# yangdongchao/RSTnet

Hardware: AMD Instinct MI355X
Metric: codec+LM audio frames/sec (24 kHz, 12.5 Hz tokens) at batch=1 and batch=64; RVQ code-index exact-match (higher is better)
Workload: dtype f32 (large GEMMs: operands as three bf16 planes, six bf16 matrix-instruction products per fp32 product, f32 accumulate); 1 GPU; MimiCodec encode->RVQ(8x2048x256)->decode, BASELINE.json configs[1]; batch_per_gpu=64, weights=random-init (rstnet_amd.synth seed 0), parallelism=replica x1, utterances sharded, RCCL weight broadcast only

## Files before the change

### rstnet_amd/csrc/b3_common.h

```cpp
#pragma once
#include "rst_common.h"

typedef short bf16x8 __attribute__((ext_vector_type(8)));
typedef unsigned u32x2 __attribute__((ext_vector_type(2)));
typedef unsigned u32x4 __attribute__((ext_vector_type(4)));
typedef float f32x2 __attribute__((ext_vector_type(2)));
typedef __bf16 bf16x2_t __attribute__((ext_vector_type(2)));

__device__ __forceinline__ unsigned b3_peel(f32x2& v) {
    const unsigned h = __builtin_bit_cast(unsigned, __builtin_convertvector(v, bf16x2_t));
    v[0] -= __uint_as_float(h << 16);
    v[1] -= __uint_as_float(h & 0xffff0000u);
    return h;
}

constexpr int B3_SH_ROWS = 128;

struct B3SharedTile {
    int b, t0;
    long m0, mlim;
};
struct B3SharedRow {
    unsigned ao;
    int klo, kn;
};

__host__ __device__ __forceinline__ constexpr int b3_shared_step(int R) { return B3_SH_ROWS - (R - 1); }
__host__ __device__ __forceinline__ constexpr int b3_shared_tiles_per_utt(int T_out, int R) { return (T_out + b3_shared_step(R) - 1) / b3_shared_step(R); }

__host__ __device__ __forceinline__ B3SharedTile b3_shared_tile(int mt, int R, int T_out) {
    const int tpu = b3_shared_tiles_per_utt(T_out, R), step = b3_shared_step(R);
    B3SharedTile t;
    t.b = mt / tpu;
    t.t0 = (mt - t.b * tpu) * step;
    t.m0 = (long)t.b * T_out + t.t0;
    t.mlim = (long)t.b * T_out + (t.t0 + step < T_out ? t.t0 + step : T_out);
    return t;
}

__host__ __device__ __forceinline__ B3SharedRow b3_shared_row(const B3SharedTile& t, int r, int R, int G, int TC, long x_bstride, int lk) {
    const long g = (long)t.t0 + r - (R - 1);
    const long f0 = g * G;
    B3SharedRow o;
    o.klo = 0;
    if (g < 0 || f0 >= TC) {
        o.kn = 0;
        o.ao = (unsigned)(lk * 4);
    } else {
        const long left = TC - f0;
        o.kn = (int)((left < G ? left : (long)G) / 16);
        o.ao = (unsigned)(((long)t.b * x_bstride + f0 + lk) * 4);
    }
    return o;
}

__host__ __device__ __forceinline__ unsigned b3_shared_load_offset(const B3SharedRow& row, int kt, bool& ok) {
    ok = (unsigned)kt < (unsigned)row.kn;
    return row.ao + (ok ? (unsigned)kt : 0u) * 64u;
}

#define B3_QA {2, 0, 1, 1, 0, 0}
#define B3_QB {0, 2, 1, 0, 1, 0}
```

### rstnet_amd/csrc/gemm_win.hip

```cpp
#include <algorithm>
#include "rst_common.h"
#include "rst_kernels.h"
#include "b3_common.h"

namespace {

constexpr int BK = 32;

template <int TM, int TN, bool FULL = false>
__device__ __forceinline__ void gw_epilogue(const GemmWinParams& p, const f32x16 (&acc)[TM][TN], int m0w, int n0w, int M, int lane) {
    const bool has_res = p.res != nullptr;
#pragma unroll
    for (int j = 0; j < TN; ++j) {
        const int n = n0w + j * 32 + (lane & 31);
        const bool n_ok = FULL || n < p.N;
        const float bias = (p.bias && n_ok) ? p.bias[n] : 0.0f;
        const float scale = (p.scale && n_ok) ? p.scale[n] : 1.0f;
#pragma unroll
        for (int i = 0; i < TM; ++i) {
            const int mb = m0w + i * 32 + 4 * (lane >> 5);
            const long o = (long)mb * p.ldy + n;
            float r[16];
#pragma unroll
            for (int e = 0; e < 16; ++e) {
                const int dm = (e & 3) + 8 * (e >> 2);
                r[e] = (has_res && n_ok && (FULL || mb + dm < M)) ? p.res[o + (long)dm * p.ldy] : 0.0f;
            }
#pragma unroll
            for (int e = 0; e < 16; ++e) {
                const int dm = (e & 3) + 8 * (e >> 2);
                float v = acc[i][j][e] + bias;
                if (p.act_out == 1) v = rst_gelu(v);
                if (has_res) v = r[e] + scale * v;
                if (p.act_out == 2) v = rst_elu(v);
                if (n_ok && (FULL || mb + dm < M)) p.y[o + (long)dm * p.ldy] = v;
            }
        }
    }
}

template <int TM, int TN, int WM, int WN, bool VEC, bool ELU, int KB, bool FAST>
__device__ __forceinline__ void gw_tile(const GemmWinParams& p, const int tile, const int m0, const int n0, float* smem) {
    constexpr int BM = 32 * TM * WM;
    constexpr int BN = 32 * TN * WN;
    constexpr int LDS_LD = KB + 4;
    constexpr int RP = 1024 / KB;
    constexpr int RA = BM / RP;
    constexpr int RB = BN / RP;
    static_assert(BM % RP == 0 && BN % RP == 0, "tile smaller than one staging pass");
    float* As = smem;
    float* Bs = smem + 2 * BM * LDS_LD;

    const int tid = threadIdx.x;
    const int lane = tid & 63;
    const int wave = tid >> 6;
    const int wm = wave / WN, wn = wave % WN;

    const int M = p.B * p.T_out;
    const int TC = p.T_in * p.C;
    const int PC = p.P * p.C;

    const int lrow = tid / (KB / 4);
    const int lk = (tid % (KB / 4)) * 4;
    long a_off[RA];
    long h_off[RA];
    int a_f0[RA];
    int a_klo[RA], a_khi[RA];
    bool a_ok[RA];
#pragma unroll
    for (int j = 0; j < RA; ++j) {
        const int m = m0 + lrow + RP * j;
        a_ok[j] = m < M;
        const int mm = a_ok[j] ? m : 0;
        const int b = mm / p.T_out;
        const int t = mm - b * p.T_out;
        a_off[j] = (long)b * p.x_bstride;
        h_off[j] = (long)b * PC;
        a_f0[j] = (t * p.S - p.P) * p.C;
        a_klo[j] = a_ok[j] ? max(0, -a_f0[j]) : 0x7fffffff;
        a_khi[j] = a_ok[j] ? min(p.K, TC - a_f0[j]) : 0;
    }

    f32x4 ra[RA], rb[RB];

    auto load_elem_a = [&](int j, int f) -> float {
        float v = 0.0f;
        if (f >= 0) {
            if (f < TC) v = p.x[a_off[j] + f];
            else if (p.pad_mode == 1) v = p.x[a_off[j] + TC - p.C + f % p.C];
        } else if (p.hist) {
            v = p.hist[h_off[j] + PC + f];
        } else if (p.pad_mode == 1) {
            int c = f % p.C;
            if (c < 0) c += p.C;
            v = p.x[a_off[j] + c];
        }
        return v;
    };

    typedef int i32x4 __attribute__((ext_vector_type(4)));
    int ma[RA], mb[RB];
    auto masked_load = [&](const float* src, bool ok, int& m) -> f32x4 {
        m = ok ? -1 : 0;
        asm volatile("" : "+v"(m));
        return *reinterpret_cast<const f32x4*>(ok ? src : p.w);
    };
    auto apply_mask = [&](const f32x4 v, const int m) -> f32x4 {
        const i32x4 b = __builtin_bit_cast(i32x4, v) & m;
        return __builtin_bit_cast(f32x4, b);
    };
    auto load_tiles = [&](int kt) {
        const int k = kt * KB + lk;
#pragma unroll
        for (int j = 0; j < RA; ++j) {
            if (VEC) {
                const int f = a_f0[j] + k;
                bool ok = a_ok[j] && k < p.K;
                const float* src = p.x + a_off[j] + f;
                if (f < 0) {
                    if (p.hist) {
                        src = p.hist + h_off[j] + PC + f;
                    } else if (p.pad_mode == 1) {
                        int c = f % p.C;
                        if (c < 0) c += p.C;
                        src = p.x + a_off[j] + c;
                    } else {
                        ok = false;
                    }
                } else if (f >= TC) {
                    if (p.pad_mode == 1) src = p.x + a_off[j] + TC - p.C + f % p.C;
                    else ok = false;
                }
                ra[j] = masked_load(src, ok, ma[j]);
            } else {
                ma[j] = -1;
                f32x4 v = {0.f, 0.f, 0.f, 0.f};
                if (a_ok[j]) {
#pragma unroll
                    for (int e = 0; e < 4; ++e)
                        if (k + e < p.K) v[e] = load_elem_a(j, a_f0[j] + k + e);
                }
                ra[j] = v;
            }
        }
#pragma unroll
        for (int j = 0; j < RB; ++j) {
            const int n = n0 + lrow + RP * j;
            const float* wp = p.w + (long)n * p.K + k;
            if (VEC) {
                rb[j] = masked_load(wp, n < p.N && k < p.K, mb[j]);
            } else {
                mb[j] = -1;
                f32x4 v = {0.f, 0.f, 0.f, 0.f};
                if (n < p.N) {
#pragma unroll
                    for (int e = 0; e < 4; ++e)
                        if (k + e < p.K) v[e] = wp[e];
                }
                rb[j] = v;
            }
        }
    };

    auto store_tiles = [&](int buf, const bool masked = true) {
        float* a = As + buf * BM * LDS_LD;
        float* b = Bs + buf * BN * LDS_LD;
#pragma unroll
        for (int j = 0; j < RA; ++j) {
            f32x4 v = (VEC && masked) ? apply_mask(ra[j], ma[j]) : ra[j];
            if (ELU) {
                v[0] = rst_elu(v[0]); v[1] = rst_elu(v[1]); v[2] = rst_elu(v[2]); v[3] = rst_elu(v[3]);
            }
            *reinterpret_cast<f32x4*>(a + (lrow + RP * j) * LDS_LD + lk) = v;
        }
#pragma unroll
        for (int j = 0; j < RB; ++j)
            *reinterpret_cast<f32x4*>(b + (lrow + RP * j) * LDS_LD + lk) = (VEC && masked) ? apply_mask(rb[j], mb[j]) : rb[j];
    };

    f32x16 acc[TM][TN];
#pragma unroll
    for (int i = 0; i < TM; ++i)
#pragma unroll
        for (int j = 0; j < TN; ++j)
#pragma unroll
            for (int e = 0; e < 16; ++e) acc[i][j][e] = 0.0f;

    const int nk_all = (p.K + KB - 1) / KB;
    const int nsplit = FAST ? (int)gridDim.y : 1;
    const int per_split = (nk_all + nsplit - 1) / nsplit;
// ... 159 lines not shown
    const int tiles_n = (p.N + BN - 1) / BN;
    const int nk = p.K / KB;
    const bool k_ok = p.K % KB == 0;

    const int xcd = blockIdx.x & 7;
    const int first = gw_xcd_first(tiles, xcd);
    const int count = gw_xcd_first(tiles, xcd + 1) - first;
    const int stride = ((int)gridDim.x + 7 - xcd) >> 3;
    int l = blockIdx.x >> 3;
    if (l >= count) return;

    struct Ctx {
        const float* ap[RA];
        unsigned bo[RB];
    };
    auto setup = [&](int m0, int n0, Ctx& c) -> bool {
        bool interior = k_ok && m0 + BM <= M && n0 + BN <= p.N;
#pragma unroll
        for (int j = 0; j < RA; ++j) {
            const int m = min(m0 + lrow + RP * j, M - 1);
            const int b = m / p.T_out;
            const int t = m - b * p.T_out;
            const int f0 = (t * p.S - p.P) * p.C;
            interior = interior && f0 >= 0 && f0 + p.K <= TC;
            c.ap[j] = p.x + (long)b * p.x_bstride + f0 + lk;
        }
#pragma unroll
        for (int j = 0; j < RB; ++j) c.bo[j] = (unsigned)min(n0 + lrow + RP * j, p.N - 1) * (unsigned)p.K + lk;
        return __syncthreads_and(interior);
    };

    f32x4 ra[RA], rb[RB];
    auto issue = [&](const Ctx& c, int kt) {
#pragma unroll
        for (int j = 0; j < RA; ++j) ra[j] = *reinterpret_cast<const f32x4*>(c.ap[j] + kt * KB);
#pragma unroll
        for (int j = 0; j < RB; ++j) rb[j] = *reinterpret_cast<const f32x4*>(p.w + c.bo[j] + kt * KB);
    };
    auto store_tiles = [&](int buf) {
        float* a = As + buf * BM * LDS_LD;
        float* b = Bs + buf * BN * LDS_LD;
#pragma unroll
        for (int j = 0; j < RA; ++j) {
            f32x4 v = ra[j];
            if (ELU) {
                v[0] = rst_elu(v[0]); v[1] = rst_elu(v[1]); v[2] = rst_elu(v[2]); v[3] = rst_elu(v[3]);
            }
            *reinterpret_cast<f32x4*>(a + (lrow + RP * j) * LDS_LD + lk) = v;
        }
#pragma unroll
        for (int j = 0; j < RB; ++j)
            *reinterpret_cast<f32x4*>(b + (lrow + RP * j) * LDS_LD + lk) = rb[j];
    };

    f32x16 acc[TM][TN];
    auto clear = [&]() {
#pragma unroll
        for (int i = 0; i < TM; ++i)
#pragma unroll
            for (int j = 0; j < TN; ++j)
#pragma unroll
                for (int e = 0; e < 16; ++e) acc[i][j][e] = 0.0f;
    };
    auto mma_tile = [&](int buf, int ks0, int ks1) {
        const float* a = As + buf * BM * LDS_LD + (wm * TM * 32 + frag_row) * LDS_LD + frag_k;
        const float* b = Bs + buf * BN * LDS_LD + (wn * TN * 32 + frag_row) * LDS_LD + frag_k;
#pragma unroll
        for (int ks = ks0; ks < ks1; ++ks) {
            f32x4 fa[TM], fb[TN];
#pragma unroll
            for (int i = 0; i < TM; ++i) fa[i] = *reinterpret_cast<const f32x4*>(a + i * 32 * LDS_LD + ks * 8);
#pragma unroll
            for (int j = 0; j < TN; ++j) fb[j] = *reinterpret_cast<const f32x4*>(b + j * 32 * LDS_LD + ks * 8);
#pragma unroll
            for (int e = 0; e < 4; ++e)
#pragma unroll
                for (int i = 0; i < TM; ++i)
#pragma unroll
                    for (int j = 0; j < TN; ++j)
                        acc[i][j] = __builtin_amdgcn_mfma_f32_32x32x2f32(fa[i][e], fb[j][e], acc[i][j], 0, 0, 0);
        }
    };
    auto step = [&](const Ctx& c, int kt, int buf) {
        if (DBG == 5) {
#pragma unroll
            for (int e = 0; e < 4 * (KB / 8); ++e)
#pragma unroll
                for (int i = 0; i < TM; ++i)
#pragma unroll
                    for (int j = 0; j < TN; ++j)
                        acc[i][j] = __builtin_amdgcn_mfma_f32_32x32x2f32(ra[0][e & 3], rb[0][e & 3], acc[i][j], 0, 0, 0);
            return;
        }
        store_tiles(buf ^ 1);
        if (DBG != 1) issue(c, kt);
        __builtin_amdgcn_sched_barrier(0);
        mma_tile(buf, 0, KB / 8);
        __syncthreads();
    };
    auto prime = [&](const Ctx& c, int buf) {
        issue(c, 0);
        store_tiles(buf);
        issue(c, 1);
        __syncthreads();
    };

    Ctx c, cn;
    int tile = first + l;
    int m0 = (tile / tiles_n) * BM, n0 = (tile % tiles_n) * BN;
    bool fast = nk >= 2 && setup(m0, n0, c);
    int buf = 0;
    if (fast) prime(c, 0);
    for (;;) {
        const bool has_next = l + stride < count;
        const int tile_n = tile + stride;
        const int m0n = (tile_n / tiles_n) * BM, n0n = (tile_n % tiles_n) * BN;
        bool fast_n = false;
        if (fast) {
            clear();
            int lkt = 2;
            for (int kt = 0; kt < nk; ++kt) {
                if (lkt == nk) {
                    lkt = 0;
                    if (has_next) {
                        fast_n = setup(m0n, n0n, cn);
                        if (fast_n) c = cn;
                    }
                }
                step(c, lkt, buf);
                ++lkt;
                buf ^= 1;
            }
            gw_epilogue<TM, TN, true>(p, acc, m0 + wm * TM * 32, n0 + wn * TN * 32, M, lane);
        } else {
            gw_tile<TM, TN, WM, WN, true, ELU, KB, false>(p, tile, m0, n0, smem);
            if (has_next) fast_n = nk >= 2 && setup(m0n, n0n, c);
        }
        if (!has_next) break;
        if (fast_n && !fast) prime(c, buf);
        fast = fast_n;
        l += stride;
        tile = tile_n;
        m0 = m0n;
        n0 = n0n;
    }
}


constexpr int B3_SETS_A = 4;
constexpr int B3_SETS_B = 2;
constexpr int B3_KB = 16;
constexpr int B3_RS = 24;
constexpr int B3_WTILE = 3 * 128 * B3_KB;

template <int V>
struct b3_int { static constexpr int value = V; };

__host__ __device__ __forceinline__ constexpr int b3_row(int g) { return (g & ~7) | (2 * (g & 3) + ((g >> 2) & 1)); }
__host__ __device__ __forceinline__ constexpr int b3_slot(int r) { return (r & ~7) | (((r & 7) >> 1) + 4 * (r & 1)); }

template <bool ELU, bool MASK, int NWN, int DBG = 0, bool BUFL = true, bool DIRW = false>
__global__ __launch_bounds__(128 * NWN) __attribute__((amdgpu_waves_per_eu(2, 2))) void gemm_win_b3_stream_kernel(const GemmWinParams p, const int tiles) {
    constexpr int TM = 2, TN = 2;
    constexpr int NT = 128 * NWN;
    constexpr int BM = 128, BN = 64 * NWN;
    constexpr int RA = 512 / NT;
    constexpr int A_PLANE = BM * B3_RS, W_PLANE = DIRW ? 0 : BN * B3_RS;
    constexpr int BUF = 3 * (A_PLANE + W_PLANE);
    constexpr int NSA = B3_SETS_A, NSB = B3_SETS_B;
    static_assert(NSA == 4 && NSB == 2, "the rotation below is written out for four activation sets and two weight sets");
    static_assert(NWN == 2 || NWN == 4, "two or four waves along N");
    extern __shared__ __attribute__((aligned(16))) float smem[];
    short* const lds = reinterpret_cast<short*>(smem);

    const int tid = threadIdx.x;
    const int lane = tid & 63;
    const int wave = tid >> 6;
    const int wm = wave / NWN, wn = wave % NWN;
    const int lrow = b3_row(tid >> 2);
    const int lk = (tid & 3) * 4;
    const int frag_row = lane & 31;
    const int frag_k = (lane >> 5) * 8;

    const int M = p.B * p.T_out;
    const int TC = p.T_in * p.C;
    const int tiles_n = (p.N + BN - 1) / BN;
    const int nk = p.K / B3_KB;

    const int xcd = blockIdx.x & 7;
    const int first = gw_xcd_first(tiles, xcd);
    const int count = gw_xcd_first(tiles, xcd + 1) - first;
    const int stride = ((int)gridDim.x + 7 - xcd) >> 3;
    int l = blockIdx.x >> 3;
    if (l >= count) return;

    struct Ctx {
        unsigned ao[RA];
        int klo[RA], kn[RA];
    };
    auto setup = [&](int m0, Ctx& c) {
#pragma unroll
        for (int j = 0; j < RA; ++j) {
            const int m = m0 + lrow + (NT / 4) * j;
            const int mm = min(m, M - 1);
            const int b = mm / p.T_out;
            const int t = mm - b * p.T_out;
            const int f0 = (t * p.S - p.P) * p.C;
            long off = (long)b * p.x_bstride + f0 + lk;
            if (MASK) {
                int klo = max(0, -f0) / B3_KB, khi = min(p.K, TC - f0) / B3_KB;
                if (m >= M || klo >= khi) {
                    klo = khi = 0;
                    off = lk;
                }
                c.klo[j] = klo;
                c.kn[j] = khi - klo;
                off += (long)klo * B3_KB;
            }
            c.ao[j] = (unsigned)(off * 4);
        }
    };
    auto w_tile = [&](int n0) {
        return DIRW ? (unsigned)(n0 / 32) * (unsigned)nk * 3072u : (unsigned)(n0 / 128) * (unsigned)nk * (unsigned)(B3_WTILE * 2);
    };
    const unsigned wo = DIRW ? (unsigned)(wn * TN) * (unsigned)nk * 3072u + (unsigned)lane * 16u
                             : (unsigned)(((long)(tid >> 8) * nk * B3_WTILE + (tid & 255) * 8) * 2);
    const unsigned wo_blk = (unsigned)nk * 3072u;

    f32x4 ra[NSA][RA];
    int rm[NSA][RA];
    u32x4 rb[NSB][3];
    u32x4 rw[NSB][TN][3];
    const int a_dst = lrow * B3_RS + lk;
    const int b_dst = 3 * A_PLANE + ((tid >> 8) * 128 + b3_row((tid & 255) >> 1)) * B3_RS + (tid & 1) * 8;
    const int a_frag = (wm * TM * 32 + frag_row) * B3_RS + frag_k;
    const int b_frag = 3 * A_PLANE + (wn * TN * 32 + frag_row) * B3_RS + frag_k;

    const __amdgpu_buffer_rsrc_t rs_x = __builtin_amdgcn_make_buffer_rsrc(const_cast<float*>(p.x), 0, 0xffffffff, 0x00020000);
    const __amdgpu_buffer_rsrc_t rs_w = __builtin_amdgcn_make_buffer_rsrc(const_cast<short*>(p.w3), 0, 0xffffffff, 0x00020000);
    auto load_a = [&](auto MM, const Ctx& c, const int kt, f32x4 (&dst)[RA], int (&mask)[RA]) {
        constexpr bool MK = decltype(MM)::value != 0;
#pragma unroll
        for (int j = 0; j < RA; ++j) {
            if (MK) {
                const unsigned d = (unsigned)(kt - c.klo[j]);
                const bool ok = d < (unsigned)c.kn[j];
                mask[j] = ok ? -1 : 0;
                const unsigned vo = c.ao[j] + (ok ? d : 0u) * (B3_KB * 4);
                if (BUFL) dst[j] = __builtin_bit_cast(f32x4, __builtin_amdgcn_raw_buffer_load_b128(rs_x, vo, 0, 0));
                else dst[j] = *reinterpret_cast<const f32x4*>(reinterpret_cast<const char*>(p.x) + vo);
            } else {
                if (BUFL) dst[j] = __builtin_bit_cast(f32x4, __builtin_amdgcn_raw_buffer_load_b128(rs_x, c.ao[j], kt * (B3_KB * 4), 0));
                else dst[j] = *reinterpret_cast<const f32x4*>(reinterpret_cast<const char*>(p.x) + (long)kt * (B3_KB * 4) + c.ao[j]);
            }
        }
    };
    auto load_w = [&](const unsigned wb, const int kt, u32x4 (&dst)[3]) {
#pragma unroll
        for (int q = 0; q < 3; ++q) {
            const unsigned so = wb + (unsigned)kt * (B3_WTILE * 2) + q * (128 * B3_KB * 2);
            if (BUFL) dst[q] = __builtin_amdgcn_raw_buffer_load_b128(rs_w, wo, so, 0);
            else dst[q] = *reinterpret_cast<const u32x4*>(reinterpret_cast<const char*>(p.w3) + so + wo);
        }
    };
    auto load_wq = [&](auto UU, auto QQ, const unsigned wb, const int kt) {
        constexpr int U = decltype(UU)::value, q = decltype(QQ)::value;
#pragma unroll
        for (int j = 0; j < TN; ++j) {
            const unsigned so = wb + (unsigned)kt * 3072u + q * 1024u;
            if (BUFL) rw[U][j][q] = __builtin_amdgcn_raw_buffer_load_b128(rs_w, wo + j * wo_blk, so, 0);
            else rw[U][j][q] = *reinterpret_cast<const u32x4*>(reinterpret_cast<const char*>(p.w3) + so + wo + j * wo_blk);
        }
    };
    auto take_a = [&](auto MM, const f32x4 src, const int mask, f32x2 (&v)[2]) {
        typedef int i32x4 __attribute__((ext_vector_type(4)));
        f32x4 x = src;
        if (decltype(MM)::value != 0) x = __builtin_bit_cast(f32x4, __builtin_bit_cast(i32x4, x) & mask);
        if (ELU) {
            x[0] = rst_elu(x[0]); x[1] = rst_elu(x[1]); x[2] = rst_elu(x[2]); x[3] = rst_elu(x[3]);
        }
        v[0] = f32x2{x[0], x[1]};
        v[1] = f32x2{x[2], x[3]};
    };

    f32x16 acc[TM][TN];
    auto clear = [&]() {
#pragma unroll
        for (int i = 0; i < TM; ++i)
#pragma unroll
            for (int j = 0; j < TN; ++j)
#pragma unroll
                for (int e = 0; e < 16; ++e) acc[i][j][e] = 0.0f;
    };

    auto stage = [&](auto SS, auto MM, const Ctx& c, const int kta, const unsigned bp, const int ktb, const int buf) {
        constexpr int S = decltype(SS)::value;
        constexpr int F = (S + 3) % 4, SB = S % 2, FB = (S + 1) % 2;
        if (DBG != 2 && DBG != 3) {
            if (!DIRW) {
                load_w(bp, ktb, rb[FB]);
                __builtin_amdgcn_sched_barrier(0);
            }
            load_a(MM, c, kta, ra[F], rm[F]);
        }
        bf16x8 fa[TM][3], fb[TN][3];
        const short* rd = lds + buf * BUF;
        short* wr = lds + (buf ^ 1) * BUF;
        constexpr int QA[6] = {2, DIRW ? 1 : 0, DIRW ? 0 : 1, DIRW ? 0 : 1, DIRW ? 1 : 0, 0};
        constexpr int QB[6] = {0, DIRW ? 0 : 2, DIRW ? 0 : 1, DIRW ? 2 : 0, 1, DIRW ? 1 : 0};
        if (DIRW && DBG != 3) {
#pragma unroll
            for (int i = 0; i < TM; ++i) fa[i][2] = *reinterpret_cast<const bf16x8*>(rd + a_frag + 2 * A_PLANE + i * 32 * B3_RS);
#pragma unroll
            for (int i = 0; i < TM; ++i) fa[i][1] = *reinterpret_cast<const bf16x8*>(rd + a_frag + A_PLANE + i * 32 * B3_RS);
#pragma unroll
            for (int i = 0; i < TM; ++i) fa[i][0] = *reinterpret_cast<const bf16x8*>(rd + a_frag + i * 32 * B3_RS);
        } else if (DBG != 3) {
#pragma unroll
            for (int j = 0; j < TN; ++j) fb[j][0] = *reinterpret_cast<const bf16x8*>(rd + b_frag + j * 32 * B3_RS);
#pragma unroll
            for (int i = 0; i < TM; ++i) fa[i][2] = *reinterpret_cast<const bf16x8*>(rd + a_frag + 2 * A_PLANE + i * 32 * B3_RS);
#pragma unroll
            for (int i = 0; i < TM; ++i) fa[i][0] = *reinterpret_cast<const bf16x8*>(rd + a_frag + i * 32 * B3_RS);
#pragma unroll
            for (int j = 0; j < TN; ++j) fb[j][2] = *reinterpret_cast<const bf16x8*>(rd + b_frag + 2 * W_PLANE + j * 32 * B3_RS);
#pragma unroll
            for (int i = 0; i < TM; ++i) fa[i][1] = *reinterpret_cast<const bf16x8*>(rd + a_frag + A_PLANE + i * 32 * B3_RS);
#pragma unroll
            for (int j = 0; j < TN; ++j) fb[j][1] = *reinterpret_cast<const bf16x8*>(rd + b_frag + W_PLANE + j * 32 * B3_RS);
        } else {
#pragma unroll
            for (int q = 0; q < 3; ++q) {
#pragma unroll
                for (int i = 0; i < TM; ++i) fa[i][q] = __builtin_bit_cast(bf16x8, ra[S][0]);
#pragma unroll
                for (int jj = 0; jj < TN; ++jj) fb[jj][q] = __builtin_bit_cast(bf16x8, rb[SB][q]);
            }
        }
        __builtin_amdgcn_sched_barrier(0);

        f32x2 v[RA][2];
        u32x2 h[RA];
        constexpr bool SIDE = DBG != 1 && DBG != 3;
        constexpr int PB = 2 * RA + 1, WOPS = DIRW ? 0 : 3, NOPS = WOPS + 3 * PB;
#pragma unroll
        for (int m = 0; m < 24; ++m) {
            const int t = m >> 2, i = (m >> 1) & 1, j = m & 1;
            if (DIRW && DBG != 3) acc[i][j] = __builtin_amdgcn_mfma_f32_32x32x16_bf16(fa[i][QA[t]], __builtin_bit_cast(bf16x8, rw[SB][j][QB[t]]), acc[i][j], 0, 0, 0);
            else acc[i][j] = __builtin_amdgcn_mfma_f32_32x32x16_bf16(fa[i][QA[t]], fb[j][QB[t]], acc[i][j], 0, 0, 0);
            if (DIRW && DBG != 2 && DBG != 3) {
                if (m == 11) load_wq(b3_int<SB>{}, b3_int<0>{}, bp, ktb);
                if (m == 15) load_wq(b3_int<SB>{}, b3_int<2>{}, bp, ktb);
                if (m == 23) load_wq(b3_int<SB>{}, b3_int<1>{}, bp, ktb);
            }
            if (SIDE && m == 0) {
#pragma unroll
                for (int r = 0; r < RA; ++r) take_a(MM, ra[S][r], rm[S][r], v[r]);
            }
            const int op = RA == 2 ? m - 1 : ((m & 1) ? (m - 1) >> 1 : -1);
            if (SIDE && op >= 0 && op < NOPS) {
                if (op < WOPS) {
                    *reinterpret_cast<u32x4*>(wr + b_dst + op * W_PLANE) = rb[SB][op];
                } else {
                    const int u = op - WOPS;
                    const int q = u / PB, w = u % PB;
                    if (w < 2 * RA) {
                        if (DBG == 5) h[w >> 1][w & 1] = __builtin_bit_cast(unsigned, v[w >> 1][w & 1][0]) + q;
                        else h[w >> 1][w & 1] = b3_peel(v[w >> 1][w & 1]);
                    } else {
#pragma unroll
                        for (int r = 0; r < RA; ++r) *reinterpret_cast<u32x2*>(wr + a_dst + q * A_PLANE + r * (NT / 4) * B3_RS) = h[r];
                    }
                }
            }
            __builtin_amdgcn_sched_barrier(0);
        }
        if (DBG != 4) __syncthreads();
    };

    auto prime = [&](const Ctx& c, const unsigned bp, int buf) {
        short* wr = lds + buf * BUF;
        {
            f32x4 xa[RA];
            int xm[RA];
            u32x4 xb[3];
            load_a(b3_int<MASK>{}, c, 0, xa, xm);
            if (!DIRW) load_w(bp, 0, xb);
#pragma unroll
            for (int j = 0; j < RA; ++j) {
                f32x2 v[2];
                take_a(b3_int<MASK>{}, xa[j], xm[j], v);
#pragma unroll
                for (int q = 0; q < 3; ++q) {
                    u32x2 hh;
                    hh[0] = b3_peel(v[0]);
                    hh[1] = b3_peel(v[1]);
                    *reinterpret_cast<u32x2*>(wr + a_dst + q * A_PLANE + j * (NT / 4) * B3_RS) = hh;
                }
            }
            if (!DIRW) {
#pragma unroll
                for (int q = 0; q < 3; ++q) *reinterpret_cast<u32x4*>(wr + b_dst + q * W_PLANE) = xb[q];
            }
        }
        if (DIRW) {
            load_wq(b3_int<0>{}, b3_int<0>{}, bp, 0); load_wq(b3_int<0>{}, b3_int<2>{}, bp, 0); load_wq(b3_int<0>{}, b3_int<1>{}, bp, 0);
            load_wq(b3_int<1>{}, b3_int<0>{}, bp, 1); load_wq(b3_int<1>{}, b3_int<2>{}, bp, 1); load_wq(b3_int<1>{}, b3_int<1>{}, bp, 1);
        } else {
            load_w(bp, 1, rb[0]);
        }
#pragma unroll
        for (int g = 1; g < 4; ++g) load_a(b3_int<MASK>{}, c, g, ra[g - 1], rm[g - 1]);
        __syncthreads();
    };

    Ctx c;
    int tile = first + l;
    int m0 = (tile / tiles_n) * BM, n0 = (tile % tiles_n) * BN;
    setup(m0, c);
    unsigned bp = w_tile(n0);
    unsigned bpn = bp;
    int kb = 2;
    prime(c, bp, 0);
    for (;;) {
        const int ln = l + stride;
        const bool has_next = ln < count;
        const int tile_n = first + ln;
        const int m0n = (tile_n / tiles_n) * BM, n0n = (tile_n % tiles_n) * BN;
        clear();
        int kf = 4;
        auto cross = [&]() {
            kf = 0;
            if (has_next) {
                setup(m0n, c);
                bpn = w_tile(n0n);
            }
// ... 239 lines not shown
#pragma unroll
        for (int g = 1; g < 4; ++g) load_a(c, g, ra[g - 1], rm[g - 1]);
        __syncthreads();
    }
    for (;;) {
        const int ln = l + stride;
        const bool has_next = ln < count;
        const int tile_n = first + ln;
        const B3SharedTile ti = b3_shared_tile(tile / tiles_n, R, p.T_out);
        clear();
        int kf = 4;
        for (int kt = 0; kt < nkg; kt += 4) {
            if (kf == nkg) {
                kf = 0;
                if (has_next) {
                    setup(tile_n, c);
                    bpn = w_tile((tile_n % tiles_n) * BN);
                }
            }
            stage(b3_int<0>{}, c, kf, bp, bpn, kt, 0);
            stage(b3_int<1>{}, c, kf + 1, bp, bpn, kt + 1, 1);
            stage(b3_int<2>{}, c, kf + 2, bp, bpn, kt + 2, 0);
            stage(b3_int<3>{}, c, kf + 3, bp, bpn, kt + 3, 1);
            kf += 4;
        }
        bp = bpn;
        if (n0 + BN <= p.N) gw_epilogue_rows<TM, TN>(p, acc, ti.m0, (int)(ti.mlim - ti.m0), wm * TM * 32, n0 + wn * TN * 32, lane);
        else gw_epilogue<TM, TN, false>(p, acc, (int)ti.m0 + wm * TM * 32, n0 + wn * TN * 32, (int)ti.mlim, lane);
        if (!has_next) break;
        l = ln;
        tile = tile_n;
        n0 = (tile % tiles_n) * BN;
    }
}

template <bool DIRW>
__global__ __launch_bounds__(256) void gemm_win_b3_pack_kernel(const float* __restrict__ w, short* __restrict__ w3, int N, int K, long total) {
    const long i = (long)blockIdx.x * 256 + threadIdx.x;
    if (i >= total) return;
    const int kq = K / 4;
    const int n = (int)(i / kq);
    const int k = (int)(i % kq) * 4;
    f32x4 v = {0.f, 0.f, 0.f, 0.f};
    if (n < N) v = *reinterpret_cast<const f32x4*>(w + (long)n * K + k);
    f32x2 v0 = {v[0], v[1]}, v1 = {v[2], v[3]};
    short* dst = DIRW ? w3 + ((long)(n / 32) * (K / B3_KB) + k / B3_KB) * (3 * 512) + ((n % 32) + 32 * ((k % B3_KB) / 8)) * 8 + k % 8
                      : w3 + ((long)(n / 128) * (K / B3_KB) + k / B3_KB) * B3_WTILE + b3_slot(n % 128) * B3_KB + k % B3_KB;
#pragma unroll
    for (int q = 0; q < 3; ++q) {
        u32x2 h;
        h[0] = b3_peel(v0);
        h[1] = b3_peel(v1);
        *reinterpret_cast<u32x2*>(dst + q * (DIRW ? 512 : 128 * B3_KB)) = h;
    }
}

static bool b3_dirw() {
    static const int v = rst_knob("RST_B3_DIRW", 1);
    return v != 0;
}

template <int TM, int TN, int WM, int WN, int KB = BK>
int launch_cfg(const GemmWinParams& p, bool vec, hipStream_t stream) {
    constexpr int BM = 32 * TM * WM, BN = 32 * TN * WN;
    const long M = (long)p.B * p.T_out;
    const long tiles = ((M + BM - 1) / BM) * ((p.N + BN - 1) / BN);
    if (tiles <= 0) return RST_OK;
    if (tiles > 0x7fffffffL) {
        rst_set_error("gemm_win: too many tiles (%ld)", tiles);
        return RST_ERR_UNSUPPORTED;
    }
    const size_t lds = 2 * (BM + BN) * (KB + 4) * sizeof(float);
    auto go = [&](auto k) {
        constexpr auto kern = decltype(k)::fn;
        rst_allow_dynamic_lds<kern>(128 * 1024);
        hipLaunchKernelGGL(kern, dim3((unsigned)tiles, (unsigned)(p.split_k > 1 ? p.split_k : 1)), dim3(256), lds, stream, p);
    };
    const bool elu = p.act_in == 1;
    if (vec && elu) go(RstKernel<gemm_win_kernel<TM, TN, WM, WN, true, true, KB>>{});
    else if (vec) go(RstKernel<gemm_win_kernel<TM, TN, WM, WN, true, false, KB>>{});
    else if (elu) go(RstKernel<gemm_win_kernel<TM, TN, WM, WN, false, true, KB>>{});
    else go(RstKernel<gemm_win_kernel<TM, TN, WM, WN, false, false, KB>>{});
    return rst_check_launch("gemm_win");
}

static int gw_cu_count() {
    return rst_cu_count();
}

template <int KB>
int launch_stream(const GemmWinParams& p, long tiles, hipStream_t stream) {
    if (tiles > 0x7fffffffL) {
        rst_set_error("gemm_win: too many tiles (%ld)", tiles);
        return RST_ERR_UNSUPPORTED;
    }
    const size_t lds = 2 * (128 + 128) * (KB + 4) * sizeof(float);
    static const int per_cu_env = rst_knob("RST_GEMM_STREAM_WGS", 0);
    const int per_cu = per_cu_env > 0 ? per_cu_env : (KB == 16 ? 3 : 2);
    const long resident = (long)per_cu * gw_cu_count();
    const unsigned grid = (unsigned)(tiles < resident ? tiles : resident);
    auto go = [&](auto k) {
        constexpr auto kern = decltype(k)::fn;
        rst_allow_dynamic_lds<kern>(128 * 1024);
        hipLaunchKernelGGL(kern, dim3(grid), dim3(256), lds, stream, p, (int)tiles);
    };
#ifdef RST_ABLATION
    static const int dbg = rst_knob("RST_GEMM_DBG", 0);
    if (KB == 16 && dbg == 1) { go(RstKernel<gemm_win_stream_kernel<false, 16, 1>>{}); return rst_check_launch("gemm_win"); }
    if (KB == 16 && dbg == 5) { go(RstKernel<gemm_win_stream_kernel<false, 16, 5>>{}); return rst_check_launch("gemm_win"); }
#endif
    if (p.act_in == 1) go(RstKernel<gemm_win_stream_kernel<true, KB>>{});
    else go(RstKernel<gemm_win_stream_kernel<false, KB>>{});
    return rst_check_launch("gemm_win");
}

static int b3_shared_taps(const GemmWinParams& p) {
    const long G = (long)p.S * p.C;
    if (G % 64 != 0 || p.K % G != 0) return 0;
    const long R = p.K / G;
    if ((R != 2 && R != 3) || p.P != (R - 1) * p.S) return 0;
    return (int)R;
}

template <int NWN, int R>
int launch_shared_b3_cfg(const GemmWinParams& p, hipStream_t stream) {
    constexpr int BN = 64 * NWN;
    const long tiles = (long)p.B * b3_shared_tiles_per_utt(p.T_out, R) * ((p.N + BN - 1) / BN);
    if (tiles > 0x7fffffffL) {
        rst_set_error("gemm_win: too many tiles (%ld)", tiles);
        return RST_ERR_UNSUPPORTED;
    }
    const size_t lds = 2 * 3 * (B3_SH_ROWS + R - 1) * B3_RS * sizeof(short);
    const long resident = (long)(NWN == 2 ? 2 : 1) * gw_cu_count();
    const unsigned grid = (unsigned)(tiles < resident ? tiles : resident);
    if (p.act_in == 1) hipLaunchKernelGGL((gemm_win_b3_stream_shared_kernel<true, NWN, R>), dim3(grid), dim3(128 * NWN), lds, stream, p, (int)tiles);
    else hipLaunchKernelGGL((gemm_win_b3_stream_shared_kernel<false, NWN, R>), dim3(grid), dim3(128 * NWN), lds, stream, p, (int)tiles);
    return rst_check_launch("gemm_win_b3");
}

template <int NWN>
int launch_stream_b3_cfg(const GemmWinParams& p, hipStream_t stream) {
    constexpr int BN = 64 * NWN;
    const long M = (long)p.B * p.T_out;
    const long tiles = ((M + 127) / 128) * ((p.N + BN - 1) / BN);
    if (tiles > 0x7fffffffL) {
        rst_set_error("gemm_win: too many tiles (%ld)", tiles);
        return RST_ERR_UNSUPPORTED;
    }
    const bool dirw = b3_dirw();
    const size_t lds = 2 * 3 * (128 + (dirw ? 0 : BN)) * B3_RS * sizeof(short);
    static const int per_cu = rst_knob("RST_B3_WGS", NWN == 2 ? 2 : 1);
    const long resident = (long)per_cu * gw_cu_count();
    const unsigned grid = (unsigned)(tiles < resident ? tiles : resident);
    auto go = [&](auto k) {
        constexpr auto kern = decltype(k)::fn;
        rst_allow_dynamic_lds<kern>(128 * 1024);
        hipLaunchKernelGGL(kern, dim3(grid), dim3(128 * NWN), lds, stream, p, (int)tiles);
    };
    bool lean = p.P == 0 && M % 128 == 0 && p.N % BN == 0 && (long)(p.T_out - 1) * p.S * p.C + p.K <= (long)p.T_in * p.C;
#ifdef RST_ABLATION
    static const int force_mask = rst_knob("RST_B3_FORCE_MASK", 0);
    if (force_mask) lean = false;
    static const int dbg = rst_knob("RST_B3_DBG", 0);
    if (dirw && dbg == 1) { go(RstKernel<gemm_win_b3_stream_kernel<false, true, NWN, 1, true, true>>{}); return rst_check_launch("gemm_win_b3"); }
    if (dirw && dbg == 2) { go(RstKernel<gemm_win_b3_stream_kernel<false, true, NWN, 2, true, true>>{}); return rst_check_launch("gemm_win_b3"); }
    if (dirw && dbg == 3) { go(RstKernel<gemm_win_b3_stream_kernel<false, true, NWN, 3, true, true>>{}); return rst_check_launch("gemm_win_b3"); }
    if (dirw && dbg == 4) { go(RstKernel<gemm_win_b3_stream_kernel<false, true, NWN, 4, true, true>>{}); return rst_check_launch("gemm_win_b3"); }
    if (dirw && dbg == 5) { go(RstKernel<gemm_win_b3_stream_kernel<false, true, NWN, 5, true, true>>{}); return rst_check_launch("gemm_win_b3"); }
    static const int bufl = rst_knob("RST_B3_BUF", 1);
    if (!bufl && dirw && p.act_in != 1) {
        if (lean) go(RstKernel<gemm_win_b3_stream_kernel<false, false, NWN, 0, false, true>>{});
        else go(RstKernel<gemm_win_b3_stream_kernel<false, true, NWN, 0, false, true>>{});
        return rst_check_launch("gemm_win_b3");
    }
#endif
#ifdef RST_ABLATION
    if (!dirw) {
        if (p.act_in == 1) {
            if (lean) go(RstKernel<gemm_win_b3_stream_kernel<true, false, NWN>>{});
            else go(RstKernel<gemm_win_b3_stream_kernel<true, true, NWN>>{});
        } else {
            if (lean) go(RstKernel<gemm_win_b3_stream_kernel<false, false, NWN>>{});
            else go(RstKernel<gemm_win_b3_stream_kernel<false, true, NWN>>{});
        }
        return rst_check_launch("gemm_win_b3");
    }
#endif
    static const int share = rst_knob("RST_B3_SHARE", 1);
    if (share) {
        const int taps = b3_shared_taps(p);
        if (taps == 2) return launch_shared_b3_cfg<NWN, 2>(p, stream);
        if (taps == 3) return launch_shared_b3_cfg<NWN, 3>(p, stream);
    }
    if (p.act_in == 1) {
        if (lean) go(RstKernel<gemm_win_b3_stream_kernel<true, false, NWN, 0, true, true>>{});
        else go(RstKernel<gemm_win_b3_stream_kernel<true, true, NWN, 0, true, true>>{});
    } else {
        if (lean) go(RstKernel<gemm_win_b3_stream_kernel<false, false, NWN, 0, true, true>>{});
        else go(RstKernel<gemm_win_b3_stream_kernel<false, true, NWN, 0, true, true>>{});
    }
    return rst_check_launch("gemm_win_b3");
}

int launch_stream_b3(const GemmWinParams& p, hipStream_t stream) {
    static const int wide_knob = rst_knob("RST_B3_WIDE", 1);
    const int waste = ((p.N + 255) / 256) * 256 - p.N;
    const long wide_tiles = (((long)p.B * p.T_out + 127) / 128) * ((p.N + 255) / 256);
    if (wide_knob && p.N >= 256 && waste * 8 <= p.N && wide_tiles >= 2L * gw_cu_count()) return launch_stream_b3_cfg<4>(p, stream);
    return launch_stream_b3_cfg<2>(p, stream);
}

}

static int gw_tile_cfg(long M, int N) {
    if (N > 64) return M > 4096 ? 0 : 1;
    if (N > 32) return 2;
    return 3;
}
static void gw_tile_dims(int cfg, int& BM, int& BN) {
    BM = cfg == 0 ? 128 : cfg == 1 ? 32 : cfg == 2 ? 128 : 256;
    BN = cfg == 0 ? 128 : cfg == 1 ? 128 : cfg == 2 ? 64 : 32;
}

int rst_gemm_split_plan_impl(long M, int N, int K) {
    if (M <= 0 || M > 4096 || (M <= 32 && N <= 64)) return 1;
    int BM, BN;
    gw_tile_dims(gw_tile_cfg(M, N), BM, BN);
    const long tiles = ((M + BM - 1) / BM) * ((N + BN - 1) / BN);
    const int nk = (K + BK - 1) / BK;
    int s = 1;
    while (tiles * s * 2 <= 256 && nk / (2 * s) >= 2 && s < 64) s *= 2;
    return s;
}

bool rst_gemm_win_b3_shape_ok(int B, int T_in, int T_out, int C, int K, int N, int pad_mode, long x_bstride, bool has_hist) {
    if (B <= 0 || T_in <= 0 || T_out <= 0 || C <= 0 || K <= 0 || N <= 0) return false;
    const long M = (long)B * T_out;
    if (gw_tile_cfg(M, N) != 0) return false;
    if (K % 64 != 0 || C % 16 != 0 || x_bstride % 4 != 0 || has_hist || pad_mode != 0) return false;
    const long x_bytes = ((long)(B - 1) * x_bstride + (long)T_in * C) * 4;
    const long w_bytes = rst_gemm_win_b3_weight_elems_impl(N, K) * 2;
    return x_bytes < 0xfffff000L && w_bytes < 0xfffff000L;
}

int rst_launch_gemm_win(const GemmWinParams& p, hipStream_t stream) {
    RST_REQUIRE(p.B >= 0 && p.T_in >= 0 && p.T_out >= 0 && p.C > 0 && p.K > 0 && p.N > 0 && p.S > 0 && p.P >= 0,
                "gemm_win: bad sizes B=%d T_in=%d T_out=%d C=%d K=%d N=%d S=%d P=%d", p.B, p.T_in, p.T_out, p.C,
                p.K, p.N, p.S, p.P);
    if (p.B == 0 || p.T_out == 0) return RST_OK;
    RST_REQUIRE(p.w && p.y && (p.x || p.T_in == 0), "gemm_win: null pointer");
    RST_REQUIRE((long)p.T_in * p.C < 0x7fffffffL && (long)p.T_out * p.S * p.C < 0x7fffffffL,
                "gemm_win: per-batch activation too large for 32-bit indexing");
    const bool vec = (p.C % 4 == 0) && (p.K % 4 == 0) && (p.x_bstride % 4 == 0) &&
                     ((uintptr_t)p.x % 16 == 0) && ((uintptr_t)p.w % 16 == 0) &&
                     (!p.hist || (uintptr_t)p.hist % 16 == 0);
    const long M = (long)p.B * p.T_out;
    RST_REQUIRE(p.split_k <= 1 || (p.ws && p.counters && M <= 4096), "gemm_win: split-K needs M <= 4096 and the scratch buffers");
    RST_REQUIRE(!p.w3 || gw_tile_cfg(M, p.N) == 0, "gemm_win_b3: %ld x %d is not a large-launch shape (more than 4096 rows, N > 64)", M, p.N);
    switch (gw_tile_cfg(M, p.N)) {
        case 0: {
            const long tiles = ((M + 127) / 128) * ((p.N + 127) / 128);
            static const bool kb32_only = rst_knob("RST_GEMM_KB32", 0) != 0;
            static const bool stream_off = rst_knob("RST_GEMM_STREAM", 1) == 0;
            if (p.w3) {
                RST_REQUIRE(vec && p.split_k <= 1 && (uintptr_t)p.w3 % 16 == 0 &&
                            rst_gemm_win_b3_shape_ok(p.B, p.T_in, p.T_out, p.C, p.K, p.N, p.pad_mode, p.x_bstride, p.hist != nullptr),
                            "gemm_win_b3: shape / alignment not served by the three-plane kernel (B=%d T_in=%d T_out=%d C=%d K=%d N=%d pad=%d "
                            "hist=%d); ask rst_gemm_win_b3_supported", p.B, p.T_in, p.T_out, p.C, p.K, p.N, p.pad_mode, p.hist != nullptr);
                return launch_stream_b3(p, stream);
            }
            static const int under_knob = rst_knob("RST_GEMM_UNDERFILL", 1);
            if (under_knob && tiles < gw_cu_count() && p.split_k <= 1) return launch_cfg<1, 1, 1, 4>(p, vec, stream);
            if (vec && !stream_off && p.split_k <= 1) {
                if (tiles >= 768 && !kb32_only) return launch_stream<16>(p, tiles, stream);
                return launch_stream<32>(p, tiles, stream);
            }
            if (tiles >= 768 && !kb32_only) return launch_cfg<2, 2, 2, 2, 16>(p, vec, stream);
            return launch_cfg<2, 2, 2, 2>(p, vec, stream);
        }
        case 1: return launch_cfg<1, 1, 1, 4>(p, vec, stream);
        case 2: return launch_cfg<1, 2, 4, 1>(p, vec, stream);
        default: return launch_cfg<2, 1, 4, 1>(p, vec, stream);
    }
}

int rst_gemm_split_tiles_impl(long M, int N) {
    int BM, BN;
    gw_tile_dims(gw_tile_cfg(M, N), BM, BN);
    return (int)(((M + BM - 1) / BM) * ((N + BN - 1) / BN));
}

long rst_gemm_win_b3_weight_elems_impl(int N, int K) { return (long)((N + 255) / 256) * 256 * K * 3; }

int rst_launch_gemm_win_b3_pack(const float* w, unsigned short* w3, int N, int K, hipStream_t stream) {
    RST_REQUIRE(w && w3 && N > 0 && K > 0 && K % 16 == 0, "gemm_win_b3_pack_weight: bad arguments (K %% 16 == 0 required, N=%d K=%d)", N, K);
    RST_REQUIRE((uintptr_t)w % 16 == 0 && (uintptr_t)w3 % 16 == 0, "gemm_win_b3_pack_weight: pointers must be 16-byte aligned");
    const long total = (long)((N + 255) / 256) * 256 * (K / 4);
#ifdef RST_ABLATION
    if (!b3_dirw()) {
        hipLaunchKernelGGL(gemm_win_b3_pack_kernel<false>, dim3((unsigned)((total + 255) / 256)), dim3(256), 0, stream, w, reinterpret_cast<short*>(w3), N, K, total);
        return rst_check_launch("gemm_win_b3_pack_weight");
    }
#endif
    hipLaunchKernelGGL(gemm_win_b3_pack_kernel<true>, dim3((unsigned)((total + 255) / 256)), dim3(256), 0, stream, w, reinterpret_cast<short*>(w3), N, K, total);
    return rst_check_launch("gemm_win_b3_pack_weight");
}
```

Before: 196,200 frames/s.

## Add 16x16x32 bf16 MFMA variant of the streaming three-plane GEMM kernel

Adds an MI=16 path to the windowed b3 streaming GEMM that uses 16x16x32 bf16 matrix instructions instead of the 32x32 form. It comes with a new LDS layout with XOR swizzling, new row and weight fragment indexing, and a dedicated epilogue. The path is chosen by default for lean shapes with K >= 512, and its interleaved schedule overlaps weight loads and A-plane peeling with the MFMAs. The aim is higher matrix-instruction throughput and lower LDS footprint per block. The cost is a large amount of hand-scheduled code and a risk of register pressure or indexing errors.

Measured after the change: 197,500 frames/s (median of 6 runs). Within noise of the previous version (+0.6%).

```diff
diff --git a/rstnet_amd/csrc/b3_common.h b/rstnet_amd/csrc/b3_common.h
--- a/rstnet_amd/csrc/b3_common.h
+++ b/rstnet_amd/csrc/b3_common.h
@@ -59,5 +59,18 @@
     return row.ao + (ok ? (unsigned)kt : 0u) * 64u;
 }
 
+__host__ __device__ __forceinline__ constexpr int b3_mi16_lds_offset(int row, int k) {
+    return row * 64 + (((k >> 3) ^ ((row >> 1) & 2)) * 16) + (k & 7) * 2;
+}
+__host__ __device__ __forceinline__ constexpr int b3_mi16_row(int g) { return (g & ~6) | ((g & 2) << 1) | ((g & 4) >> 1); }
+__host__ __device__ __forceinline__ constexpr int b3_mi16_frag_row(int lane) { return lane & 15; }
+__host__ __device__ __forceinline__ constexpr int b3_mi16_frag_k(int lane) { return 8 * (lane >> 4); }
+__host__ __device__ __forceinline__ constexpr long b3_mi16_weight_index(int nk, int b, int t, int q, int c, int lane) {
+    const int g = lane >> 4;
+    return (((long)b * nk + 2 * t + (g >> 1)) * 3 + q) * 512 + (16 * c + (lane & 15) + 32 * (g & 1)) * 8;
+}
+__host__ __device__ __forceinline__ constexpr int b3_mi16_acc_row(int lane, int e) { return 4 * (lane >> 4) + e; }
+__host__ __device__ __forceinline__ constexpr int b3_mi16_acc_col(int lane) { return lane & 15; }
+
 #define B3_QA {2, 0, 1, 1, 0, 0}
 #define B3_QB {0, 2, 1, 0, 1, 0}
diff --git a/rstnet_amd/csrc/gemm_win.hip b/rstnet_amd/csrc/gemm_win.hip
--- a/rstnet_amd/csrc/gemm_win.hip
+++ b/rstnet_amd/csrc/gemm_win.hip
@@ -36,6 +36,35 @@
                 if (n_ok && (FULL || mb + dm < M)) p.y[o + (long)dm * p.ldy] = v;
             }
         }
+    }
+}
+
+template <bool FULL>
+__device__ __forceinline__ void gw_epilogue16(const GemmWinParams& p, const f32x4 (&acc)[4][4], int m0w, int n0w, int M, int lane) {
+    const bool has_res = p.res != nullptr;
+#pragma unroll
+    for (int j = 0; j < 4; ++j) {
+        const int n = n0w + j * 16 + b3_mi16_acc_col(lane);
+        const bool n_ok = FULL || n < p.N;
+        const float bias = (p.bias && n_ok) ? p.bias[n] : 0.0f;
+        const float scale = (p.scale && n_ok) ? p.scale[n] : 1.0f;
+        const int mb = m0w + b3_mi16_acc_row(lane, 0);
+        const long o = (long)mb * p.ldy + n;
+        float r[4][4];
+#pragma unroll
+        for (int i = 0; i < 4; ++i)
+#pragma unroll
+            for (int e = 0; e < 4; ++e) r[i][e] = (has_res && n_ok && (FULL || mb + i * 16 + e < M)) ? p.res[o + (long)(i * 16 + e) * p.ldy] : 0.0f;
+#pragma unroll
+        for (int i = 0; i < 4; ++i)
+#pragma unroll
+            for (int e = 0; e < 4; ++e) {
+                float v = acc[i][j][e] + bias;
+                if (p.act_out == 1) v = rst_gelu(v);
+                if (has_res) v = r[i][e] + scale * v;
+                if (p.act_out == 2) v = rst_elu(v);
+                if (n_ok && (FULL || mb + i * 16 + e < M)) p.y[o + (long)(i * 16 + e) * p.ldy] = v;
+            }
     }
 }
 
@@ -501,14 +530,22 @@
 constexpr int B3_KB = 16;
 constexpr int B3_RS = 24;
 constexpr int B3_WTILE = 3 * 128 * B3_KB;
+constexpr int B3_MI16_MIN_K = 512;
 
 template <int V>
 struct b3_int { static constexpr int value = V; };
+template <int N, class F>
+__device__ __forceinline__ void b3_static_for(F&& f) {
+    if constexpr (N > 0) {
+        b3_static_for<N - 1>(f);
+        f(b3_int<N - 1>{});
+    }
+}
 
 __host__ __device__ __forceinline__ constexpr int b3_row(int g) { return (g & ~7) | (2 * (g & 3) + ((g >> 2) & 1)); }
 __host__ __device__ __forceinline__ constexpr int b3_slot(int r) { return (r & ~7) | (((r & 7) >> 1) + 4 * (r & 1)); }
 
-template <bool ELU, bool MASK, int NWN, int DBG = 0, bool BUFL = true, bool DIRW = false>
+template <bool ELU, bool MASK, int NWN, int DBG = 0, bool BUFL = true, bool DIRW = false, int MI = 32>
 __global__ __launch_bounds__(128 * NWN) __attribute__((amdgpu_waves_per_eu(2, 2))) void gemm_win_b3_stream_kernel(const GemmWinParams p, const int tiles) {
     constexpr int TM = 2, TN = 2;
     constexpr int NT = 128 * NWN;
@@ -526,7 +563,7 @@
     const int lane = tid & 63;
     const int wave = tid >> 6;
     const int wm = wave / NWN, wn = wave % NWN;
-    const int lrow = b3_row(tid >> 2);
+    const int lrow = MI == 16 ? b3_mi16_row(tid >> 2) : b3_row(tid >> 2);
     const int lk = (tid & 3) * 4;
     const int frag_row = lane & 31;
     const int frag_k = (lane >> 5) * 8;
@@ -631,6 +668,147 @@
         v[0] = f32x2{x[0], x[1]};
         v[1] = f32x2{x[2], x[3]};
     };
+
+    if constexpr (MI == 16) {
+        static_assert(DIRW && BUFL && DBG == 0, "the 16x16x32 form exists for the shipped configuration only");
+        constexpr int PLANE16 = BM * 64, BUF16 = 3 * PLANE16;
+        char* const ldsb = reinterpret_cast<char*>(smem);
+        const int a_dst16 = b3_mi16_lds_offset(lrow, lk);
+        const int a_frag16 = b3_mi16_lds_offset(wm * 64 + b3_mi16_frag_row(lane), b3_mi16_frag_k(lane));
+        const unsigned wo16 = (unsigned)(wn * 2) * (unsigned)nk * 3072u + (unsigned)(lane >> 5) * 3072u + (unsigned)((lane & 15) + 32 * ((lane >> 4) & 1)) * 16u;
+        u32x4 rw16[4][3];
+        auto load_w16 = [&](auto JJ, auto QQ, const unsigned wb, const int kt) {
+            constexpr int j = decltype(JJ)::value, q = decltype(QQ)::value;
+            rw16[j][q] = __builtin_amdgcn_raw_buffer_load_b128(rs_w, wo16 + (j >> 1) * wo_blk + (j & 1) * 256u, wb + (unsigned)kt * 3072u + q * 1024u, 0);
+        };
+        f32x4 acc16[4][4];
+        auto stage16 = [&](auto SS, auto MM, const Ctx& c, const int kta, const unsigned bpw, const int ktb, const int buf) {
+            constexpr int S = decltype(SS)::value;
+            constexpr int F = (S + 2) % 4;
+            load_a(MM, c, kta, ra[F], rm[F]);
+            load_a(MM, c, kta + 1, ra[F + 1], rm[F + 1]);
+            const char* rd = ldsb + buf * BUF16;
+            char* wr = ldsb + (buf ^ 1) * BUF16;
+            bf16x8 fa[4][3];
+#pragma unroll
+            for (int i = 0; i < 4; ++i) fa[i][0] = *reinterpret_cast<const bf16x8*>(rd + a_frag16 + i * 1024);
+#pragma unroll
+            for (int i = 0; i < 4; ++i) fa[i][1] = *reinterpret_cast<const bf16x8*>(rd + a_frag16 + PLANE16 + i * 1024);
+            __builtin_amdgcn_sched_barrier(0);
+            constexpr int QA[6] = {0, 0, 0, 1, 1, 2};
+            constexpr int QB[6] = {2, 1, 0, 0, 1, 0};
+            f32x2 v[RA][2];
+            u32x2 h[RA];
+            constexpr int PB = 2 * RA + 1, NOPS1 = 3 * PB, STEP = 90 / (2 * NOPS1);
+            b3_static_for<96>([&](auto M_) {
+                constexpr int m = decltype(M_)::value;
+                constexpr int t = m >> 4, j = (m >> 2) & 3, i = m & 3;
+                constexpr int qa = QA[t], qb = QB[t];
+                acc16[i][j] = __builtin_amdgcn_mfma_f32_16x16x32_bf16(fa[i][qa], __builtin_bit_cast(bf16x8, rw16[j][qb]), acc16[i][j], 0, 0, 0);
+                if constexpr (i == 3 && t == 0) load_w16(b3_int<j>{}, b3_int<2>{}, bpw, ktb);
+                if constexpr (i == 3 && t == 4) load_w16(b3_int<j>{}, b3_int<1>{}, bpw, ktb);
+                if constexpr (i == 3 && t == 5) load_w16(b3_int<j>{}, b3_int<0>{}, bpw, ktb);
+                if constexpr (m == 47) {
+#pragma unroll
+                    for (int ii = 0; ii < 4; ++ii) fa[ii][2] = *reinterpret_cast<const bf16x8*>(rd + a_frag16 + 2 * PLANE16 + ii * 1024);
+                }
+                if constexpr (m == 0 || m == NOPS1 * STEP) {
+                    constexpr int hh = m ? 1 : 0;
+#pragma unroll
+                    for (int r = 0; r < RA; ++r) take_a(MM, ra[S + hh][r], rm[S + hh][r], v[r]);
+                }
+                constexpr int s = m - 1;
+                if constexpr (s >= 0 && s % STEP == 0 && s / STEP < 2 * NOPS1) {
+                    constexpr int op = s / STEP, hh = op / NOPS1, u = op % NOPS1, q = u / PB, w = u % PB;
+                    if constexpr (w < 2 * RA) {
+                        h[w >> 1][w & 1] = b3_peel(v[w >> 1][w & 1]);
+                    } else {
+#pragma unroll
+                        for (int r = 0; r < RA; ++r) *reinterpret_cast<u32x2*>(wr + ((a_dst16 ^ (hh * 32)) + q * PLANE16 + r * (NT / 4) * 64)) = h[r];
+                    }
+                }
+                __builtin_amdgcn_sched_barrier(0);
+            });
+            __syncthreads();
+        };
+        auto prime16 = [&](const Ctx& c, const unsigned bpw) {
+#pragma unroll
+            for (int hh = 0; hh < 2; ++hh) {
+                f32x4 xa[RA];
+                int xm[RA];
+                load_a(b3_int<MASK>{}, c, hh, xa, xm);
+#pragma unroll
+                for (int j = 0; j < RA; ++j) {
+                    f32x2 v[2];
+                    take_a(b3_int<MASK>{}, xa[j], xm[j], v);
+#pragma unroll
+                    for (int q = 0; q < 3; ++q) {
+                        u32x2 hv;
+                        hv[0] = b3_peel(v[0]);
+                        hv[1] = b3_peel(v[1]);
+                        *reinterpret_cast<u32x2*>(ldsb + ((a_dst16 ^ (hh * 32)) + q * PLANE16 + j * (NT / 4) * 64)) = hv;
+                    }
+                }
+            }
+            load_w16(b3_int<0>{}, b3_int<2>{}, bpw, 0); load_w16(b3_int<1>{}, b3_int<2>{}, bpw, 0); load_w16(b3_int<2>{}, b3_int<2>{}, bpw, 0); load_w16(b3_int<3>{}, b3_int<2>{}, bpw, 0);
+            load_w16(b3_int<0>{}, b3_int<1>{}, bpw, 0); load_w16(b3_int<1>{}, b3_int<1>{}, bpw, 0); load_w16(b3_int<2>{}, b3_int<1>{}, bpw, 0); load_w16(b3_int<3>{}, b3_int<1>{}, bpw, 0);
+            load_w16(b3_int<0>{}, b3_int<0>{}, bpw, 0); load_w16(b3_int<1>{}, b3_int<0>{}, bpw, 0); load_w16(b3_int<2>{}, b3_int<0>{}, bpw, 0); load_w16(b3_int<3>{}, b3_int<0>{}, bpw, 0);
+            load_a(b3_int<MASK>{}, c, 2, ra[0], rm[0]);
+            load_a(b3_int<MASK>{}, c, 3, ra[1], rm[1]);
+            __syncthreads();
+        };
+
+        Ctx c;
+        int tile = first + l;
+        int m0 = (tile / tiles_n) * BM, n0 = (tile % tiles_n) * BN;
+        setup(m0, c);
+        unsigned bp = w_tile(n0);
+        unsigned bpn = bp;
+        int kb = 2;
+        prime16(c, bp);
+        for (;;) {
+            const int ln = l + stride;
+            const bool has_next = ln < count;
+            const int tile_n = first + ln;
+            const int m0n = (tile_n / tiles_n) * BM, n0n = (tile_n % tiles_n) * BN;
+#pragma unroll
+            for (int i = 0; i < 4; ++i)
+#pragma unroll
+                for (int j = 0; j < 4; ++j) acc16[i][j] = f32x4{0.0f, 0.0f, 0.0f, 0.0f};
+            int kf = 4;
+            constexpr b3_int<MASK> MM{};
+            for (int kt = 0; kt < nk; kt += 4) {
+                if (kf == nk) {
+                    kf = 0;
+                    if (has_next) {
+                        setup(m0n, c);
+                        bpn = w_tile(n0n);
+                    }
+                }
+                stage16(b3_int<0>{}, MM, c, kf, bp, kb, 0);
+                kb += 2;
+                if (kb == nk) {
+                    kb = 0;
+                    bp = bpn;
+                }
+                stage16(b3_int<2>{}, MM, c, kf + 2, bp, kb, 1);
+                kb += 2;
+                if (kb == nk) {
+                    kb = 0;
+                    bp = bpn;
+                }
+                kf += 4;
+            }
+            if (!MASK || (m0 + BM <= M && n0 + BN <= p.N)) gw_epilogue16<true>(p, acc16, m0 + wm * 64, n0 + wn * 64, M, lane);
+            else gw_epilogue16<false>(p, acc16, m0 + wm * 64, n0 + wn * 64, M, lane);
+            if (!has_next) break;
+            l = ln;
+            tile = tile_n;
+            m0 = m0n;
+            n0 = n0n;
+        }
+        return;
+    }
 
     f32x16 acc[TM][TN];
     auto clear = [&]() {
@@ -1176,13 +1354,13 @@
     static const int per_cu = rst_knob("RST_B3_WGS", NWN == 2 ? 2 : 1);
     const long resident = (long)per_cu * gw_cu_count();
     const unsigned grid = (unsigned)(tiles < resident ? tiles : resident);
+    bool lean = p.P == 0 && M % 128 == 0 && p.N % BN == 0 && (long)(p.T_out - 1) * p.S * p.C + p.K <= (long)p.T_in * p.C;
+#ifdef RST_ABLATION
     auto go = [&](auto k) {
         constexpr auto kern = decltype(k)::fn;
         rst_allow_dynamic_lds<kern>(128 * 1024);
         hipLaunchKernelGGL(kern, dim3(grid), dim3(128 * NWN), lds, stream, p, (int)tiles);
     };
-    bool lean = p.P == 0 && M % 128 == 0 && p.N % BN == 0 && (long)(p.T_out - 1) * p.S * p.C + p.K <= (long)p.T_in * p.C;
-#ifdef RST_ABLATION
     static const int force_mask = rst_knob("RST_B3_FORCE_MASK", 0);
     if (force_mask) lean = false;
     static const int dbg = rst_knob("RST_B3_DBG", 0);
@@ -1216,13 +1394,30 @@
         if (taps == 2) return launch_shared_b3_cfg<NWN, 2>(p, stream);
         if (taps == 3) return launch_shared_b3_cfg<NWN, 3>(p, stream);
     }
-    if (p.act_in == 1) {
-        if (lean) go(RstKernel<gemm_win_b3_stream_kernel<true, false, NWN, 0, true, true>>{});
-        else go(RstKernel<gemm_win_b3_stream_kernel<true, true, NWN, 0, true, true>>{});
-    } else {
-        if (lean) go(RstKernel<gemm_win_b3_stream_kernel<false, false, NWN, 0, true, true>>{});
-        else go(RstKernel<gemm_win_b3_stream_kernel<false, true, NWN, 0, true, true>>{});
-    }
+    auto plain = [&](auto MI_, auto LEAN_) {
+        constexpr int MI = decltype(MI_)::value;
+        constexpr bool LEAN = decltype(LEAN_)::value != 0;
+        const size_t lds_mi = MI == 16 ? (size_t)2 * 3 * 128 * 64 : lds;
+        auto go_mi = [&](auto k) {
+            constexpr auto kern = decltype(k)::fn;
+            rst_allow_dynamic_lds<kern>(128 * 1024);
+            hipLaunchKernelGGL(kern, dim3(grid), dim3(128 * NWN), lds_mi, stream, p, (int)tiles);
+        };
+        if (p.act_in == 1) go_mi(RstKernel<gemm_win_b3_stream_kernel<true, !LEAN, NWN, 0, true, true, MI>>{});
+        else go_mi(RstKernel<gemm_win_b3_stream_kernel<false, !LEAN, NWN, 0, true, true, MI>>{});
+    };
+#ifdef RST_ABLATION
+    static const int mi_knob = rst_knob("RST_B3_MI", 0);
+    const int mi = mi_knob ? mi_knob : (lean && p.K >= B3_MI16_MIN_K ? 16 : 32);
+    if (mi == 16 && lean) plain(b3_int<16>{}, b3_int<1>{});
+    else if (mi == 16) plain(b3_int<16>{}, b3_int<0>{});
+    else if (lean) plain(b3_int<32>{}, b3_int<1>{});
+    else plain(b3_int<32>{}, b3_int<0>{});
+#else
+    if (lean && p.K >= B3_MI16_MIN_K) plain(b3_int<16>{}, b3_int<1>{});
+    else if (lean) plain(b3_int<32>{}, b3_int<1>{});
+    else plain(b3_int<32>{}, b3_int<0>{});
+#endif
     return rst_check_launch("gemm_win_b3");
 }
 
```
